# megvii-research/basedet

Measured on AMD Instinct MI355X. Metric: images/sec training RetinaNet-R50-FPN 1333x800, higher is better.
Workload: dtype bf16; 1 GPU; retinanet_r50_800x1344 train step (fwd+bwd+allreduce+SGD), DummyLoader boxes, random-init weights, inputs resident in HBM; per_gpu_batch=16, global_batch=16, parallelism=dp1

## Files before the change

### basedet_amd/_lib.py

```python
import ctypes as C
import os

import torch

_HERE = os.path.dirname(os.path.abspath(__file__))
LIB_PATH = os.environ.get("BASEDET_HIP_LIB") or os.path.join(_HERE, "lib", "libbasedet_hip.so")

BD_MAX_SEGS = 8
ABI_VERSION = 112
EPI_RELU, EPI_ADD_BEFORE, EPI_ADD_AFTER, EPI_MASK, EPI_SPARSE = 1, 2, 4, 8, 16


class BasedetHipError(RuntimeError):
    pass


class ConvDesc(C.Structure):
    _fields_ = [
        ("N", C.c_int32), ("Cin", C.c_int32), ("Cout", C.c_int32), ("R", C.c_int32), ("S", C.c_int32),
        ("stride", C.c_int32), ("pad", C.c_int32), ("nseg", C.c_int32),
        ("Hi", C.c_int32 * BD_MAX_SEGS), ("Wi", C.c_int32 * BD_MAX_SEGS),
        ("Ho", C.c_int32 * BD_MAX_SEGS), ("Wo", C.c_int32 * BD_MAX_SEGS),
        ("in_off", C.c_int32 * BD_MAX_SEGS), ("out_off", C.c_int32 * BD_MAX_SEGS),
        ("in_pix_per_img", C.c_int32), ("out_pix_per_img", C.c_int32),
        ("route", C.c_int32 * 4), ("sr_seed", C.c_uint32),
        ("gskip", C.c_int32), ("gskip_ws", C.c_void_p), ("gskip_ws_bytes", C.c_size_t),
        ("gskip_gmap", C.c_void_p), ("gskip_gmap_bytes", C.c_size_t), ("gskip_dxmap", C.c_void_p), ("gskip_dxmap_bytes", C.c_size_t),
        ("gskip_dx_clean", C.c_int32),
        ("fwd_map", C.c_void_p), ("fwd_map_bytes", C.c_size_t), ("fwd_clean", C.c_int32),
    ]


class PackDesc(C.Structure):
    _fields_ = [("w", C.c_void_p), ("row_scale", C.c_void_p), ("w_fwd", C.c_void_p), ("w_dgrad", C.c_void_p),
                ("Cout", C.c_int32), ("RS", C.c_int32), ("Cin", C.c_int32), ("block_start", C.c_int32)]


class ImageDesc(C.Structure):
    _fields_ = [("offset", C.c_int64), ("src_h", C.c_int32), ("src_w", C.c_int32), ("dst_h", C.c_int32), ("dst_w", C.c_int32),
                ("flip", C.c_int32), ("reserved_", C.c_int32 * 1)]


_P, _I, _L, _F, _Z = C.c_void_p, C.c_int, C.c_int64, C.c_float, C.c_size_t
_D = C.POINTER(ConvDesc)

SIGNATURES = {
    "bd_last_error_string": (C.c_char_p, []),
    "bd_version": (_I, []),
    "bd_conv_last_kernel": (C.c_char_p, []),
    "bd_probe_mfma_rate": (_I, [C.c_double, C.POINTER(C.c_double), C.POINTER(C.c_double), _P]),
    "bd_probe_kernel_clock": (_I, [C.c_char_p, _I, C.POINTER(C.c_double), C.POINTER(C.c_double)]),
    "bd_conv2d_fwd": (_I, [_D, _P, _P, _P, _P, _P, _I, _P]),
    "bd_conv2d_dgrad": (_I, [_D, _P, _P, _P, _P, _P, _I, _P]),
    "bd_conv2d_dgrad_gskip_bytes": (_Z, [_D]),
    "bd_conv2d_gskip_map_bytes": (_Z, [_D, _I]),
    "bd_gskip_map_scan": (_I, [_D, _I, _P, _P, _Z, _P]),
    "bd_fwd_live_map_bytes": (_Z, [_D]),
    "bd_fwd_live_maps": (_I, [_D, _P, _I, _I, C.POINTER(C.c_void_p), _Z, _I, _P]),
    "bd_conv2d_fwd_bits": (_I, [_D, _P, _P, _P, _P, _P, _P, _I, _P]),
    "bd_conv2d_fwd_ex": (_I, [_D, _P, _P, _P, _P, _P, _P, _P, _F, _I, _P]),
    "bd_conv2d_dgrad_ex": (_I, [_D, _P, _P, _P, _P, _P, _P, _P, _F, _I, _P]),
    "bd_conv2d_dgrad_bits": (_I, [_D, _P, _P, _P, _P, _P, _I, _P]),
    "bd_conv2d_wgrad_workspace_bytes": (_Z, [_D]),
    "bd_conv2d_wgrad": (_I, [_D, _P, _P, _P, _P, _I, _P, _Z, _P]),
    "bd_conv2d_wgrad_bias_workspace_bytes": (_Z, [_D]),
    "bd_conv2d_wgrad_bias": (_I, [_D, _P, _P, _P, _P, _P, _I, _P, _Z, _P]),
    "bd_fpn_deconv_pack": (_I, [_P, _I, _P, _P, _P]),
    "bd_fpn_deconv_fwd": (_I, [_P, _P, _P, _P, _I, _I, _I, _I, _I, _I, _P]),
    "bd_fpn_deconv_dgrad": (_I, [_P, _P, _P, _P, _I, _I, _I, _I, _I, _I, _P]),
    "bd_fpn_deconv_wgrad_workspace_bytes": (_Z, [_I, _I, _I, _I]),
    "bd_fpn_deconv_wgrad": (_I, [_P, _P, _P, _I, _P, _Z, _I, _I, _I, _I, _I, _I, _P]),
    "bd_wgrad_queue_create": (_I, [_P]),
    "bd_wgrad_queue_destroy": (_I, [_P]),
    "bd_wgrad_queue_pending": (_I, [_P]),
    "bd_conv2d_wgrad_queued": (_I, [_P, _D, _P, _P, _P, _P, _P, _I, _P, _Z, _P]),
    "bd_wgrad_queue_flush": (_I, [_P, _P]),
    "bd_stem_conv7x7_fwd": (_I, [_I, _I, _I, _P, _P, _P, _P, _P]),
    "bd_stem_conv7x7_raw_fwd": (_I, [_I, _I, _I, _P, _P, _P, _P]),
    "bd_stem_pool_fwd": (_I, [_I, _I, _I, _P, _P, _P, _P, _P]),
    "bd_stem_weight_pack": (_I, [_P, _P, _P, _P]),
    "bd_maxpool3x3s2_bwd": (_I, [_P, _P, _P, _I, _I, _I, _I, _P, _P]),
    "bd_stem_conv7x7_wgrad_workspace_bytes": (_Z, [_I, _I, _I]),
    "bd_stem_conv7x7_wgrad": (_I, [_I, _I, _I, _P, _P, _P, _P, _I, _P, _Z, _P]),
    "bd_weight_pack": (_I, [_P, _P, _P, _P, _I, _I, _I, _P]),
    "bd_weight_pack_blocks": (_I, [_I, _I, _I]),
    "bd_weight_pack_multi": (_I, [_P, _I, _I, _P]),
    "bd_colsum_workspace_bytes": (_Z, [_I]),
    "bd_colsum_bf16": (_I, [_P, _I, _L, _L, _L, _I, _P, _I, _P, _Z, _P]),
    "bd_pad_normalize": (_I, [_P, _I, _I, _I, _I, _I, _P, _P, _P, _P]),
    "bd_bottleneck_fwd_supported": (_I, [_I, _I, _I, _I, _I, _I, _I]),
    "bd_bottleneck_fwd": (_I, [_I, _I, _I, _I, _I, _I, _P, _P, _P, _P, _P, _P, _P, _P, _P, _P, _P]),
    "bd_h2d_create": (_I, [C.POINTER(C.c_void_p), _I, _I]),
    "bd_h2d_threads": (_I, [_P]),
    "bd_h2d_submit": (_I, [_P, _P, _I, _L, _P, _L, _P]),
    "bd_h2d_destroy": (_I, [_P]),
    "bd_pad_normalize_nchw": (_I, [_P, _I, _I, _I, _I, _I, _P, _P, _P, _P]),
    "bd_resize_pad_normalize": (_I, [_P, _L, C.POINTER(ImageDesc), _I, _I, _I, _P, _P, _P, _P]),
    "bd_maxpool3x3s2_fwd": (_I, [_P, _I, _I, _I, _I, _P, _P]),
    "bd_upsample2x_add_fwd": (_I, [_P, _L, _L, _P, _L, _L, _I, _I, _I, _I, _P]),
    "bd_upsample2x_add_bwd": (_I, [_P, _L, _L, _P, _L, _L, _I, _I, _I, _I, _I, _P]),
    "bd_relu_bf16": (_I, [_P, _P, _L, _P]),
    "bd_relu_bwd_bf16": (_I, [_P, _P, _P, _P, _L, _P]),
    "bd_add_bf16": (_I, [_P, _P, _P, _L, _P]),
    "bd_anchors_generate": (_I, [_I, _I, _I, _F, _P, _I, _P, _P]),
    "bd_points_generate": (_I, [_I, _I, _I, _F, _I, _P, _P]),
    "bd_box_pairwise": (_I, [_P, _I, _P, _I, _I, _P, _P]),
    "bd_box_encode": (_I, [_P, _P, _L, _P, _P, _P, _P]),
    "bd_box_decode": (_I, [_P, _P, _L, _P, _P, _P, _P]),
    "bd_retina_assign_encode": (_I, [_P, _I, _P, _P, _I, _I, _F, _F, _I, _P, _P, _P, _P, _P, _P, _P, _Z, _P]),
    "bd_fcos_assign": (_I, [_P, _I, _P, _P, _P, _I, _F, _P, _P, _I, _I, _P, _P, _P, _P, _P]),
    "bd_ota_assign_workspace_bytes": (_Z, [_I, _I]),
    "bd_ota_assign": (_I, [_P, _I, _P, _P, _I, _P, _I, _I, _P, _P, _P, _I, _I, _F, _F, _F, _F, _I, _P, _P, _P, _P, _P, _Z, _P]),
    "bd_ota_sinkhorn_workspace_bytes": (_Z, [_I, _I, _I]),
    "bd_ota_assign_sinkhorn": (_I, [_P, _I, _P, _P, _I, _P, _I, _I, _P, _P, _P, _I, _I, _F, _F, _F, _F, _I, _F, _I, _P, _P, _P, _P, _P, _Z, _P]),
    "bd_freeanchor_workspace_bytes": (_Z, [_I, _I, _I, _I]),
    "bd_freeanchor_loss_fwd_bwd": (_I, [_P, _I, _P, _I, _I, _P, _I, _I, _P, _P, _I, _I, _P, _P, _F, _I, _F, _F, _F, _F, _P, _P, _P, _P, _Z, _P]),
    "bd_atss_assign_workspace_bytes": (_Z, [_I, _I]),
    "bd_atss_assign": (_I, [_P, _I, _P, _P, _I, _I, _F, _P, _P, _I, _I, _P, _P, _P, _P, _P, _Z, _P]),
    "bd_nms_workspace_bytes": (_Z, [_I]),
    "bd_batched_nms": (_I, [_P, _P, _P, _I, _F, _I, _P, _P, _P, _Z, _P]),
    "bd_focal_loss_fwd_bwd": (_I, [_P, _P, _L, _I, _I, _F, _F, _P, _I, _F, _P, _P, _I, _P]),
    "bd_smooth_l1_fwd_bwd": (_I, [_P, _P, _P, _L, _I, _I, _F, _P, _I, _F, _P, _P, _P]),
    "bd_loss_grid_cap": (_I, []),
    "bd_iou_ltrb_fwd_bwd": (_I, [_P, _P, _P, _P, _L, _I, _P, _F, _P, _P, _P]),
    "bd_bce_logits_fwd_bwd": (_I, [_P, _I, _I, _P, _P, _L, _P, _P, _P, _P]),
    "bd_groupnorm_workspace_bytes": (_Z, [_I, _I, _I, _L]),
    "bd_groupnorm_fwd": (_I, [_P, _P, _P, _I, _I, _P, _P, _L, _I, _F, _I, _P, _P, _P, _Z, _P]),
    "bd_conv2d_fwd_gnstats_bytes": (_Z, [_D]),
    "bd_conv2d_fwd_gnstats": (_I, [_D, _P, _P, _P, _P, _P, _Z, _P]),
    "bd_groupnorm_fwd_parts": (_I, [_D, _P, _P, _P, _P, _F, _I, _P, _P, _P]),
    "bd_groupnorm_bwd": (_I, [_P, _P, _P, _P, _P, _I, _I, _P, _P, _L, _I, _I, _P, _P, _P, _I, _P, _Z, _P]),
    "bd_bn_workspace_bytes": (_Z, [_L, _I]),
    "bd_bn_stats_fwd": (_I, [_P, _I, _L, _L, _L, _I, _F, _F, _P, _P, _P, _P, _P, _P, _Z, _P]),
    "bd_bn_apply_act_fwd": (_I, [_P, _L, _L, _P, _P, _P, _P, _P, _L, _L, _P, _L, _L, _I, _L, _I, _I, _P]),
    "bd_bn_bwd_reduce": (_I, [_P, _L, _L, _P, _L, _L, _P, _P, _I, _L, _I, _P, _P, _P, _Z, _P]),
    "bd_bn_bwd_apply": (_I, [_P, _L, _L, _P, _L, _L, _P, _P, _P, _P, _P, _P, _P, _L, _L, _I, _L, _I, _P]),
    "bd_fcos_offsets_fwd": (_I, [_P, _I, _P, _I, _I, _P, _P, _P, _L, _P, _P]),
    "bd_fcos_offsets_workspace_bytes": (_Z, []),
    "bd_fcos_offsets_bwd": (_I, [_P, _I, _P, _I, _I, _P, _P, _P, _L, _P, _P, _P, _P, _P, _Z, _P]),
    "bd_rpn_assign_encode": (_I, [_P, _I, _P, _P, _I, _I, _F, _F, _I, _P, _P, _P, _P, _P, _P, _P, _Z, _P]),
    "bd_sample_labels": (_I, [_P, _P, _P, _I, _I, _I, _I, _P, _P]),
    "bd_segment_topk": (_I, [_P, _I, _I, _L, _I, _I, _I, _I, _P, _P, _I, _F, _I, _P, _P, _P, _P]),
    "bd_nms_batched_workspace_bytes": (_Z, [_I, _I]),
    "bd_nms_batched": (_I, [_P, _P, _P, _I, _I, _F, _I, _I, _P, _P, _P, _Z, _P]),
    "bd_rpn_proposals_workspace_bytes": (_Z, [_I, _I, _P, _I, _I, _I]),
    "bd_rpn_proposals": (_I, [_P, _I, _I, _I, _I, _I, _L, _I, _P, _P, _P, _P, _I, _P, _P, _I, _F, _I, _P, _P, _P, _Z, _I, _P]),
    "bd_rcnn_sample_targets": (_I, [_P, _P, _I, _P, _P, _I, _I, _P, _P, _I, _I, _I, _F, _F, _F, _P, _P, _P, _P, _P, _P, _P, _P]),
    "bd_roi_align_fwd": (_I, [_P, _L, _I, _I, _P, _P, _P, _P, _P, _P, _I, _I, _I, _I, _I, _P, _P]),
    "bd_conv1x1_thin_bwd_workspace_bytes": (_Z, []),
    "bd_conv1x1_thin_fwd": (_I, [_P, _P, _P, _L, _I, _I, _P, _P]),
    "bd_conv1x1_thin_bwd": (_I, [_P, _P, _P, _L, _I, _I, _P, _P, _P, _I, _P, _Z, _P]),
    "bd_roi_align_bwd": (_I, [_P, _L, _I, _I, _P, _P, _P, _P, _P, _P, _I, _I, _I, _I, _I, _P, _P]),
    "bd_roi_align_bwd_bf16_workspace_bytes": (_Z, [_I, _I, _P, _P, _I]),
    "bd_roi_align_bwd_bf16": (_I, [_P, _L, _I, _I, _I, _P, _P, _P, _P, _P, _P, _I, _I, _I, _I, _I, _P, _I, _P, _Z, _P]),
    "bd_roi_pool_fwd": (_I, [_P, _L, _I, _I, _P, _P, _P, _P, _P, _P, _I, _I, _I, _I, _P, _P]),
    "bd_roi_pool_bwd_bf16_workspace_bytes": (_Z, [_I, _I, _P, _P, _I]),
    "bd_roi_pool_bwd_bf16": (_I, [_P, _P, _L, _I, _I, _I, _P, _P, _P, _P, _P, _P, _I, _I, _I, _I, _P, _I, _P, _Z, _P]),
    "bd_subsample2x_fwd": (_I, [_P, _L, _L, _I, _I, _P, _L, _L, _I, _I, _P]),
    "bd_subsample2x_bwd_add": (_I, [_P, _L, _L, _P, _L, _L, _I, _I, _I, _I, _P]),
    "bd_f32_to_bf16": (_I, [_P, _P, _L, _P]),
    "bd_f32_to_bf16_add": (_I, [_P, _P, _L, _P]),
    "bd_rpn_loss_fwd_bwd": (_I, [_P, _I, _I, _I, _I, _P, _P, _L, _F, _P, _P, _P, _P]),
    "bd_rcnn_loss_fwd_bwd": (_I, [_P, _I, _I, _I, _P, _P, _I, _F, _P, _P, _P, _P]),
    "bd_det_scores": (_I, [_P, _I, _P, _I, _I, _L, _I, _P, _P]),
    "bd_det_select_workspace_bytes": (_Z, [_I, _I, _L, _I, _I]),
    "bd_det_select": (_I, [_P, _I, _P, _I, _I, _I, _L, _I, _I, _P, _P, _I, _F, _P, _P, _P, _P, _Z, _P]),
    "bd_rcnn_predict": (_I, [_P, _I, _I, _I, _P, _P, _I, _I, _P, _P, _P, _P, _P]),
    "bd_det_candidates": (_I, [_I, _P, _P, _P, _I, _I, _I, _P, _I, _P, _P, _L, _I, _I, _P, _P, _P, _L, _P, _P, _P, _P]),
    "bd_det_finalize": (_I, [_P, _P, _P, _P, _P, _I, _I, _I, _P, _I, _P, _P, _P, _P]),
    "bd_sgd_momentum_step": (_I, [_P, _P, _P, _L, _F, _F, _F, _F, _P]),
    "bd_ema_update": (_I, [_P, _P, _L, _F, _F, _P]),
    "bd_sgd_momentum_ema_step": (_I, [_P, _P, _P, _P, _L, _F, _F, _F, _F, _F, _F, _P]),
    "bd_swap_f32": (_I, [_P, _P, _L, _P]),
    "bd_adam_step": (_I, [_P, _P, _P, _P, _L] + [_F] * 10 + [_I, _P]),
# ... 93 lines not shown
```

### basedet_amd/csrc/bottleneck_fused.hip

```cpp
#include "common.h"

namespace {

constexpr int PH = 8, PW = 16;
constexpr int HH = PH + 2, HW = PW + 2;
constexpr int NHALO = HH * HW;
constexpr int NHP = 192;
constexpr int PITCH = 144;
constexpr int XB_BYTES = NHP * PITCH;
constexpr int W3_BYTES = 256 * PITCH;
constexpr int CMID = 64, COUT = 256;
constexpr unsigned X_NONE = 0x80000000u;

#ifdef BD_BN_STAMP
__device__ unsigned long long g_bn_stamp[16];
#define BN_STAMP(i) do { if (blockIdx.x == 0 && tid == 0 && tile_seq == 1) g_bn_stamp[i] = __builtin_amdgcn_s_memtime(); } while (0)
#else
#define BN_STAMP(i) do { } while (0)
#endif

struct BP {
    const bf16_raw *x, *w1, *w2, *w3, *wd;
    const float *b1, *b2, *b3, *bd;
    bf16_raw* y;
// ... 244 lines not shown
            for (int i = 0; i < NST; ++i) asm volatile("" : "+v"(st[a][i]));
#pragma unroll
        for (int hf = 0; hf < 2; ++hf)
#pragma unroll
        for (int half = 0; half < 2; ++half) {
            const int cbase = cb * 64 + 32 * half + 8 * q;
            const f32x4_t bv0 = *reinterpret_cast<const f32x4_t*>(B3L + cbase);
            const f32x4_t bv1 = *reinterpret_cast<const f32x4_t*>(B3L + cbase + 4);
            f32x4_t acc3[2][4], accd[2][4];
#pragma unroll
            for (int r = 0; r < 4; ++r) {
                acc3[0][r] = (f32x4_t){0.f, 0.f, 0.f, 0.f}; acc3[1][r] = (f32x4_t){0.f, 0.f, 0.f, 0.f};
                accd[0][r] = (f32x4_t){0.f, 0.f, 0.f, 0.f}; accd[1][r] = (f32x4_t){0.f, 0.f, 0.f, 0.f};
            }
#pragma unroll
            for (int ks = 0; ks < 2; ++ks) {
                bf16x8_t a[2], b[4];
#pragma unroll
                for (int t = 0; t < 2; ++t) a[t] = ld_frag_lds(W3L + (cb * 64 + (2 * half + t) * 16 + pxc) * PITCH + (ks ? xq1 : xq0));
#pragma unroll
                for (int r = 0; r < 4; ++r) b[r] = ld_frag_lds(M1 + ((hf * 4 + r) * 16 + pxc) * PITCH + (ks ? xq1 : xq0));
#pragma unroll
                for (int t = 0; t < 2; ++t)
#pragma unroll
                    for (int r = 0; r < 4; ++r) acc3[t][r] = __builtin_amdgcn_mfma_f32_16x16x32_bf16(a[t], b[r], acc3[t][r], 0, 0, 0);
                if constexpr (HAS_DS) {
#pragma unroll
                    for (int t = 0; t < 2; ++t) a[t] = ld_frag_lds(WDL + (cb * 64 + (2 * half + t) * 16 + pxc) * PITCH + (ks ? xq1 : xq0));
#pragma unroll
                    for (int r = 0; r < 4; ++r)
                        b[r] = ld_frag_lds(XB + xbuf * XB_BYTES + ((hf * 4 + r + 1) * HW + 1 + pxc) * PITCH + (ks ? xq1 : xq0));
#pragma unroll
                    for (int t = 0; t < 2; ++t)
#pragma unroll
                        for (int r = 0; r < 4; ++r) accd[t][r] = __builtin_amdgcn_mfma_f32_16x16x32_bf16(a[t], b[r], accd[t][r], 0, 0, 0);
                }
            }
            [[maybe_unused]] f32x4_t dv0, dv1;
            if constexpr (HAS_DS) {
                dv0 = *reinterpret_cast<const f32x4_t*>(B3L + 256 + cbase);
                dv1 = *reinterpret_cast<const f32x4_t*>(B3L + 256 + cbase + 4);
            }
#pragma unroll
            for (int r = 0; r < 4; ++r) {
                u32x4_t o;
#pragma unroll
                for (int k = 0; k < 4; ++k) {
                    const f32x4_t bk = (k >> 1) ? bv1 : bv0;
                    f32x2_bn_t v = {acc3[k >> 1][r][2 * (k & 1)], acc3[k >> 1][r][2 * (k & 1) + 1]};
                    v += (f32x2_bn_t){bk[2 * (k & 1)], bk[2 * (k & 1) + 1]};
                    if constexpr (!HAS_DS) {
                        const unsigned w = res_all[hf][half][r][k];
                        v += (f32x2_bn_t){bf_lo(w), bf_hi(w)};
                    } else {
                        const f32x4_t dk = (k >> 1) ? dv1 : dv0;
                        f32x2_bn_t d = {accd[k >> 1][r][2 * (k & 1)], accd[k >> 1][r][2 * (k & 1) + 1]};
                        d += (f32x2_bn_t){dk[2 * (k & 1)], dk[2 * (k & 1) + 1]};
                        const unsigned w = __builtin_bit_cast(unsigned, __builtin_convertvector(d, bf16x2_bn_t));
                        v += (f32x2_bn_t){bf_lo(w), bf_hi(w)};
                    }
                    o[k] = relu_pack2(v[0], v[1]);
                }
                __builtin_amdgcn_raw_buffer_store_b128(o, y_rsrc, yoff[hf * 4 + r], 64 * half, 0);
            }
        }

        BN_STAMP(5);
        ++tile_seq;
        if (!have_next) break;
        tile = next_tile;
#pragma unroll
        for (int i = 0; i < NST; ++i) voff[i] = nvoff[i];
        n_img = nn; ty0 = ny0; tx0 = nx0;
        next_tile = tile + stride;
        have_next = next_tile < t_end;
        if (have_next) decode(next_tile, nvoff, nn, ny0, nx0);
        if constexpr (NCH == 1) {
            if (have_next) { if ((g & 1) == 0) stage_load(st[0], nvoff, 0); else stage_load(st[1], nvoff, 0); }
            g ^= 1;
        }
    }
}

}

#ifdef BD_BN_STAMP
extern "C" int bd_debug_bn_stamp(unsigned long long* out16) {
    return hipMemcpyFromSymbol(out16, HIP_SYMBOL(g_bn_stamp), sizeof(g_bn_stamp)) == hipSuccess ? 0 : 1;
}
#endif

extern "C" int bd_bottleneck_fwd_supported(int N, int H, int W, int Cin, int Cmid, int Cout, int has_ds) {
    if (N < 1 || H < 1 || W < 1) return 0;
    if (Cmid != CMID || Cout != COUT) return 0;
    if (!((Cin == 64 && has_ds) || (Cin == 256 && !has_ds))) return 0;
    const long long bytes_in = (long long)N * H * W * Cin * 2, bytes_out = (long long)N * H * W * Cout * 2;
    return bytes_in < 0x7fffffffll && bytes_out < 0x7fffffffll;
}

extern "C" int bd_bottleneck_fwd(int N, int H, int W, int Cin, int Cmid, int Cout, const void* x, const void* w1, const float* b1,
                                 const void* w2, const float* b2, const void* w3, const float* b3, const void* wd, const float* bd,
                                 void* y, bd_stream_t stream) {
    BD_REQUIRE(x && w1 && b1 && w2 && b2 && w3 && b3 && y, "bottleneck_fwd: null pointer");
    BD_REQUIRE(bd_bottleneck_fwd_supported(N, H, W, Cin, Cmid, Cout, wd != nullptr), "bottleneck_fwd: unsupported shape N=%d %dx%d %d->%d->%d ds=%d",
               N, H, W, Cin, Cmid, Cout, wd != nullptr);
    BD_REQUIRE(wd == nullptr || bd != nullptr, "bottleneck_fwd: downsample weights without their shift");
    BP p{};
    p.x = (const bf16_raw*)x; p.w1 = (const bf16_raw*)w1; p.w2 = (const bf16_raw*)w2; p.w3 = (const bf16_raw*)w3; p.wd = (const bf16_raw*)wd;
    p.b1 = b1; p.b2 = b2; p.b3 = b3; p.bd = bd; p.y = (bf16_raw*)y;
    p.N = N; p.H = H; p.W = W;
    p.tiles_x = cdiv(W, PW);
    p.tiles_y = cdiv(H, PH);
    p.tiles_per_img = p.tiles_x * p.tiles_y;
    p.total_tiles = p.tiles_per_img * N;
    p.per_xcd = cdiv(p.total_tiles, 8);
    p.x_bytes = (unsigned)((long long)N * H * W * Cin * 2);
    p.y_bytes = (unsigned)((long long)N * H * W * Cout * 2);
    const int cus = bd_num_cus();
    int grid = (cus / 8) * 8;
    if (grid < 8) grid = 8;
    const int need = p.per_xcd * 8;
    if (grid > need) grid = need;
    const size_t lds = 2 * XB_BYTES + XB_BYTES + W3_BYTES + (wd ? W3_BYTES : 0) + BIAS_BYTES + PAD_BYTES;
    BD_ONCE_PER_DEVICE(
        (void)hipFuncSetAttribute(reinterpret_cast<const void*>(&bottleneck_fused_kernel<64, true>), hipFuncAttributeMaxDynamicSharedMemorySize,
                                  3 * XB_BYTES + 2 * W3_BYTES + BIAS_BYTES + PAD_BYTES);
        (void)hipFuncSetAttribute(reinterpret_cast<const void*>(&bottleneck_fused_kernel<256, false>), hipFuncAttributeMaxDynamicSharedMemorySize,
                                  3 * XB_BYTES + W3_BYTES + BIAS_BYTES + PAD_BYTES));
    if (wd) hipLaunchKernelGGL((bottleneck_fused_kernel<64, true>), dim3(grid), dim3(256), lds, (hipStream_t)stream, p);
    else hipLaunchKernelGGL((bottleneck_fused_kernel<256, false>), dim3(grid), dim3(256), lds, (hipStream_t)stream, p);
    BD_CHECK_LAUNCH("bd_bottleneck_fwd");
    return BD_OK;
}
```

### basedet_amd/ops.py

```python
import ctypes as C
from dataclasses import dataclass, field
from typing import List, Optional

import torch

from . import _lib
from ._lib import ConvDesc, EPI_ADD_AFTER, EPI_ADD_BEFORE, EPI_MASK, EPI_RELU, EPI_SPARSE, check, f32arr, i32arr, ptr, stream_ptr


@dataclass
class Geom:
    N: int
    H: List[int]
    W: List[int]
    off: List[int] = field(default_factory=list)
    pix_per_img: int = 0

    def __post_init__(self):
        if not self.off:
            o = 0
            self.off = []
            for h, w in zip(self.H, self.W):
                self.off.append(o)
                o += h * w
# ... 850 lines not shown
    def __init__(self):
        self._h = C.c_void_p()
        check(L().bd_wgrad_queue_create(C.byref(self._h)), "bd_wgrad_queue_create")

    def wgrad(self, d, x, g, dw, dbias, ws, row_scale=None, accumulate=False):
        check(L().bd_conv2d_wgrad_queued(self._h, C.byref(_stamp(d)), ptr(x), ptr(g), ptr(row_scale), ptr(dw), ptr(dbias), int(accumulate), ptr(ws),
                                         ws.numel() * ws.element_size(), stream_ptr()), "bd_conv2d_wgrad_queued")

    def pending(self):
        return int(L().bd_wgrad_queue_pending(self._h))

    def flush(self):
        check(L().bd_wgrad_queue_flush(self._h, stream_ptr()), "bd_wgrad_queue_flush")

    def close(self):
        if self._h:
            L().bd_wgrad_queue_destroy(self._h)
            self._h = C.c_void_p()

    def __del__(self):
        try:
            self.close()
        except Exception:
            pass


def clip_grad_value(g, lower, upper, pre_scale=1.0):
    check(L().bd_clip_grad_value(ptr(g), g.numel(), float(pre_scale), float(lower), float(upper), stream_ptr()), "bd_clip_grad_value")


def clip_grad_norm_workspace_bytes():
    return int(L().bd_clip_grad_norm_workspace_bytes())


def clip_grad_norm(g, max_norm, ord=2.0, pre_scale=1.0, norm_out=None, ws=None):
    if ws is None:
        ws = torch.empty((clip_grad_norm_workspace_bytes(),), dtype=torch.uint8, device=g.device)
    check(L().bd_clip_grad_norm(ptr(g), g.numel(), float(pre_scale), float(max_norm), float(ord), ptr(norm_out), ptr(ws), ws.numel(),
                                stream_ptr()), "bd_clip_grad_norm")
    return norm_out


class HostStager:

    _DT = {"float64": 0, "float32": 1, "uint8": 2}

    def __init__(self, device, threads=0):
        self._h = C.c_void_p()
        self.device = torch.device(device)
        index = self.device.index if self.device.index is not None else torch.cuda.current_device()
        self.device = torch.device("cuda", index)
        check(L().bd_h2d_create(C.byref(self._h), int(index), int(threads)), "bd_h2d_create")
        self.threads = int(L().bd_h2d_threads(self._h))

    def supports(self, arr):
        return hasattr(arr, "dtype") and str(arr.dtype) in self._DT and getattr(arr, "flags", None) is not None and arr.flags["C_CONTIGUOUS"]

    def submit(self, arr, out=None, chunk_elems=0):
        if out is None:
            out = torch.empty(arr.shape, dtype=torch.float32, device=self.device)
        assert out.is_contiguous() and out.numel() == arr.size and out.dtype == torch.float32
        check(L().bd_h2d_submit(self._h, C.c_void_p(arr.ctypes.data), self._DT[str(arr.dtype)], arr.size, ptr(out), int(chunk_elems),
                                stream_ptr()), "bd_h2d_submit")
        return out

    def close(self):
        if self._h:
            L().bd_h2d_destroy(self._h)
            self._h = C.c_void_p()

    def __del__(self):
        try:
            self.close()
        except Exception:
            pass


def bottleneck_fwd_supported(N, H, W, cin, cmid, cout, has_ds):
    return bool(L().bd_bottleneck_fwd_supported(int(N), int(H), int(W), int(cin), int(cmid), int(cout), int(bool(has_ds))))


def bottleneck_fwd(N, H, W, cin, cmid, cout, x, w1, b1, w2, b2, w3, b3, wd, bd, y):
    check(L().bd_bottleneck_fwd(int(N), int(H), int(W), int(cin), int(cmid), int(cout), ptr(x), ptr(w1), ptr(b1), ptr(w2), ptr(b2),
                                ptr(w3), ptr(b3), ptr(wd), ptr(bd), ptr(y), stream_ptr()), "bd_bottleneck_fwd")
    return y
```

### include/basedet_hip.h

```cpp
#ifndef BASEDET_HIP_H
#define BASEDET_HIP_H

#include <stddef.h>
#include <stdint.h>

#ifdef __cplusplus
extern "C" {
#endif

#define BD_OK 0
#define BD_EINVAL (-1)
#define BD_ELAUNCH (-2)
#define BD_EWORKSPACE (-3)

#define BD_MAX_SEGS 8

#define BD_EPI_RELU 1
#define BD_EPI_ADD_BEFORE 2
#define BD_EPI_ADD_AFTER 4
#define BD_EPI_MASK 8
#define BD_EPI_SPARSE 16

typedef void* bd_stream_t;

// ... 22 lines not shown
    int32_t fwd_clean;
} bd_conv_desc;

const char* bd_last_error_string(void);
int bd_version(void);
const char* bd_conv_last_kernel(void);
int bd_probe_mfma_rate(double seconds, double* tflops_out, double* clock_mhz_out, bd_stream_t stream);

int bd_probe_kernel_clock(const char* kernel, int reset, double* clock_mhz_out, double* busy_ms_out);


int bd_conv2d_fwd(const bd_conv_desc* d, const void* x, const void* w_packed, const float* bias,
                  const void* add, void* y, int flags, bd_stream_t stream);

int bd_conv2d_dgrad(const bd_conv_desc* d, const void* g, const void* w_packed_t, const void* add,
                    const void* mask, void* dx, int flags, bd_stream_t stream);
size_t bd_conv2d_dgrad_gskip_bytes(const bd_conv_desc* d);
size_t bd_conv2d_gskip_map_bytes(const bd_conv_desc* d, int of_dx);
int bd_gskip_map_scan(const bd_conv_desc* d, int of_dx, const void* t, void* map, size_t map_bytes, bd_stream_t stream);
size_t bd_fwd_live_map_bytes(const bd_conv_desc* d);
int bd_fwd_live_maps(const bd_conv_desc* d, const int32_t* labels, int A, int depths, void* const* maps, size_t map_bytes, int reset,
                     bd_stream_t stream);

int bd_conv2d_fwd_bits(const bd_conv_desc* d, const void* x, const void* w_packed, const float* bias, const void* add, void* y,
                       uint32_t* ybits, int flags, bd_stream_t stream);
int bd_conv2d_dgrad_bits(const bd_conv_desc* d, const void* g, const void* w_packed_t, const void* add, const uint32_t* maskbits,
                         void* dx, int flags, bd_stream_t stream);
int bd_conv2d_fwd_ex(const bd_conv_desc* d, const void* x, const void* w_packed, const float* bias, const void* add, void* y,
                     uint32_t* ybits, void* y8, float q_scale, int flags, bd_stream_t stream);
int bd_conv2d_dgrad_ex(const bd_conv_desc* d, const void* g, const void* w_packed_t, const void* add, const void* mask,
                       const uint32_t* maskbits, void* dx, void* dx8, float q_scale, int flags, bd_stream_t stream);

size_t bd_conv2d_wgrad_workspace_bytes(const bd_conv_desc* d);
int bd_conv2d_wgrad(const bd_conv_desc* d, const void* x, const void* g, const float* row_scale, float* dw,
                    int accumulate, void* ws, size_t ws_bytes, bd_stream_t stream);

size_t bd_conv2d_wgrad_bias_workspace_bytes(const bd_conv_desc* d);
int bd_conv2d_wgrad_bias(const bd_conv_desc* d, const void* x, const void* g, const float* row_scale, float* dw, float* dbias,
                         int accumulate, void* ws, size_t ws_bytes, bd_stream_t stream);

typedef struct bd_wgrad_queue* bd_wgrad_queue_t;
int bd_wgrad_queue_create(bd_wgrad_queue_t* out);
int bd_wgrad_queue_destroy(bd_wgrad_queue_t q);
int bd_wgrad_queue_pending(bd_wgrad_queue_t q);
int bd_conv2d_wgrad_queued(bd_wgrad_queue_t q, const bd_conv_desc* d, const void* x, const void* g, const float* row_scale, float* dw,
                           float* dbias, int accumulate, void* ws, size_t ws_bytes, bd_stream_t stream);
int bd_wgrad_queue_flush(bd_wgrad_queue_t q, bd_stream_t stream);



int bd_stem_conv7x7_fwd(int N, int H, int W, const void* x_halo, const void* w_stem, const float* bias,
                        void* y, bd_stream_t stream);
int bd_stem_conv7x7_raw_fwd(int N, int H, int W, const void* x_halo, const void* w_stem, void* y, bd_stream_t stream);
int bd_stem_pool_fwd(int N, int H, int W, const void* x_halo, const void* w_stem, const float* bias, void* y_pool,
                     bd_stream_t stream);
int bd_stem_weight_pack(const float* w , const float* row_scale, void* w_stem,
                        bd_stream_t stream);

int bd_maxpool3x3s2_bwd(const void* g_pool, const void* stem_out, const void* pool_out, int N, int Hs, int Ws, int C, void* g_stem,
                        bd_stream_t stream);
size_t bd_stem_conv7x7_wgrad_workspace_bytes(int N, int H, int W);
int bd_stem_conv7x7_wgrad(int N, int H, int W, const void* x_halo, const void* g_stem, const float* row_scale, float* dw, int accumulate,
                          void* ws, size_t ws_bytes, bd_stream_t stream);

int bd_weight_pack(const float* w, const float* row_scale, void* w_fwd, void* w_dgrad, int Cout, int RS,
                   int Cin, bd_stream_t stream);

typedef struct bd_pack_desc {
    const float* w;
    const float* row_scale;
    void* w_fwd;
    void* w_dgrad;
    int32_t Cout, RS, Cin, block_start;
} bd_pack_desc;
int bd_weight_pack_blocks(int Cout, int RS, int Cin);
int bd_weight_pack_multi(const bd_pack_desc* descs_dev, int n, int total_blocks, bd_stream_t stream);

size_t bd_colsum_workspace_bytes(int C);
int bd_colsum_bf16(const void* g, int N, int64_t pix_per_img, int64_t off, int64_t cnt, int C, float* out,
                   int accumulate, void* ws, size_t ws_bytes, bd_stream_t stream);

int bd_bottleneck_fwd_supported(int N, int H, int W, int Cin, int Cmid, int Cout, int has_downsample);
int bd_bottleneck_fwd(int N, int H, int W, int Cin, int Cmid, int Cout, const void* x, const void* w1, const float* b1, const void* w2,
                      const float* b2, const void* w3, const float* b3, const void* wd, const float* bd, void* y, bd_stream_t stream);


int bd_pad_normalize(const float* in, int N, int H, int W, int Hp, int Wp, const float* mean3,
                     const float* std3, void* out, bd_stream_t stream);
typedef struct bd_h2d* bd_h2d_t;
#define BD_HOST_F64 0
#define BD_HOST_F32 1
#define BD_HOST_U8 2
int bd_h2d_create(bd_h2d_t* out, int device, int threads);
int bd_h2d_threads(bd_h2d_t h);
int bd_h2d_submit(bd_h2d_t h, const void* src_host, int src_dtype, int64_t n, float* dst_dev, int64_t chunk_elems, bd_stream_t stream);
int bd_h2d_destroy(bd_h2d_t h);

int bd_pad_normalize_nchw(const float* in, int N, int H, int W, int Hp, int Wp, const float* mean3,
                          const float* std3, float* out, bd_stream_t stream);

typedef struct bd_image_desc {
    int64_t offset;
    int32_t src_h, src_w, dst_h, dst_w, flip;
    int32_t reserved_[1];
} bd_image_desc;
int bd_resize_pad_normalize(const uint8_t* packed_dev, int64_t packed_bytes, const bd_image_desc* descs_host, int N, int Hp, int Wp,
                            const float* mean3, const float* std3, void* x_halo, bd_stream_t stream);

int bd_maxpool3x3s2_fwd(const void* x, int N, int H, int W, int C, void* y, bd_stream_t stream);

int bd_upsample2x_add_fwd(const void* top, int64_t top_pix_per_img, int64_t top_off, void* lateral,
                          int64_t lat_pix_per_img, int64_t lat_off, int N, int H, int W, int C,
                          bd_stream_t stream);
int bd_upsample2x_add_bwd(const void* dlat, int64_t lat_pix_per_img, int64_t lat_off, void* dtop,
                          int64_t top_pix_per_img, int64_t top_off, int N, int H, int W, int C,
                          int accumulate, bd_stream_t stream);

int bd_fpn_deconv_pack(const float* w, int C, void* w_fwd, void* w_dgrad, bd_stream_t stream);
int bd_fpn_deconv_fwd(const void* x, const void* w_fwd, const void* add, void* y, int N, int Hc, int Wc, int Hf, int Wf, int C,
                      bd_stream_t stream);
int bd_fpn_deconv_dgrad(const void* dy, const void* w_dgrad, const void* add, void* dx, int N, int Hc, int Wc, int Hf, int Wf, int C,
                        bd_stream_t stream);
size_t bd_fpn_deconv_wgrad_workspace_bytes(int N, int Hc, int Wc, int C);
int bd_fpn_deconv_wgrad(const void* x, const void* dy, float* dw, int accumulate, void* ws, size_t ws_bytes, int N, int Hc, int Wc,
                        int Hf, int Wf, int C, bd_stream_t stream);

int bd_relu_bf16(const void* x, void* y, int64_t n, bd_stream_t stream);
int bd_relu_bwd_bf16(const void* g, const void* mask, const void* add, void* y, int64_t n, bd_stream_t stream);
int bd_add_bf16(const void* a, const void* b, void* y, int64_t n, bd_stream_t stream);


int bd_anchors_generate(int H, int W, int stride, float offset, const float* base, int A, float* out,
                        bd_stream_t stream);
int bd_points_generate(int H, int W, int stride, float offset, int A, float* out, bd_stream_t stream);

int bd_box_pairwise(const float* b1, int m, const float* b2, int n, int mode, float* out, bd_stream_t stream);

int bd_box_encode(const float* anchors, const float* gt, int64_t n, const float* mean4_host,
                  const float* std4_host, float* out, bd_stream_t stream);
int bd_box_decode(const float* anchors, const float* deltas, int64_t n, const float* mean4_host,
                  const float* std4_host, float* out, bd_stream_t stream);

int bd_retina_assign_encode(const float* anchors, int A, const float* gt_boxes, const int32_t* num_gt, int N,
                            int Gmax, float thr_lo, float thr_hi, int allow_low_quality,
                            const float* mean4_host, const float* std4_host, int32_t* labels,
                            int32_t* match_idx, float* offsets, int32_t* num_fg, void* ws, size_t ws_bytes,
                            bd_stream_t stream);

int bd_fcos_assign(const float* points, int P, const int32_t* lvl_start_host, const float* soi_host,
                   const int32_t* strides_host, int L, float radius, const float* gt_boxes,
                   const int32_t* num_gt, int N, int Gmax, int32_t* labels, float* offsets, float* ctrness,
                   float* stats, bd_stream_t stream);

size_t bd_atss_assign_workspace_bytes(int N, int P);
int bd_atss_assign(const float* points, int P, const int32_t* lvl_start_host, const int32_t* strides_host, int L, int topk,
                   float anchor_scale, const float* gt_boxes, const int32_t* num_gt, int N, int Gmax, int32_t* labels,
                   float* offsets, float* ctrness, float* stats, void* ws, size_t ws_bytes, bd_stream_t stream);

size_t bd_ota_assign_workspace_bytes(int N, int P);
int bd_ota_assign(const float* points, int P, const int32_t* lvl_start_host, const int32_t* strides_host, int L, const void* logits,
                  int K, int ld, const void* pred_ltrb, const float* gt_boxes, const int32_t* num_gt, int N, int Gmax, float alpha,
                  float gamma, float reg_weight, float center_radius, int candidate_k, int32_t* labels, float* targets,
                  float* gt_ious, float* stats, void* ws, size_t ws_bytes, bd_stream_t stream);

size_t bd_ota_sinkhorn_workspace_bytes(int N, int P, int Gmax);
int bd_ota_assign_sinkhorn(const float* points, int P, const int32_t* lvl_start_host, const int32_t* strides_host, int L,
                           const void* logits, int K, int ld, const void* pred_ltrb, const float* gt_boxes, const int32_t* num_gt,
// ... 251 lines not shown
```

Measured before the change: 727.4 images/sec.

## Add DMA-staged fused bottleneck kernel variant for layer1 non-downsample blocks

Adds a new fused layer1 bottleneck kernel for the 256-channel, no-downsample case. It stages halo input chunks straight into LDS with buffer DMA, double-buffers them, and prefetches the next tile's input during the 3x3 stage, with extra loads into a pad region to warm L2. It runs by default unless a route bit disables it, and the ABI gains a route argument. The aim is to hide input-load latency behind MFMA work and cut LDS use, at the cost of more complex synchronisation and a separate code path.

```diff
diff --git a/basedet_amd/_lib.py b/basedet_amd/_lib.py
--- a/basedet_amd/_lib.py
+++ b/basedet_amd/_lib.py
@@ -89,7 +89,7 @@
     "bd_colsum_bf16": (_I, [_P, _I, _L, _L, _L, _I, _P, _I, _P, _Z, _P]),
     "bd_pad_normalize": (_I, [_P, _I, _I, _I, _I, _I, _P, _P, _P, _P]),
     "bd_bottleneck_fwd_supported": (_I, [_I, _I, _I, _I, _I, _I, _I]),
-    "bd_bottleneck_fwd": (_I, [_I, _I, _I, _I, _I, _I, _P, _P, _P, _P, _P, _P, _P, _P, _P, _P, _P]),
+    "bd_bottleneck_fwd": (_I, [_I, _I, _I, _I, _I, _I, _P, _P, _P, _P, _P, _P, _P, _P, _P, _P, _I, _P]),
     "bd_h2d_create": (_I, [C.POINTER(C.c_void_p), _I, _I]),
     "bd_h2d_threads": (_I, [_P]),
     "bd_h2d_submit": (_I, [_P, _P, _I, _L, _P, _L, _P]),
diff --git a/basedet_amd/csrc/bottleneck_fused.hip b/basedet_amd/csrc/bottleneck_fused.hip
--- a/basedet_amd/csrc/bottleneck_fused.hip
+++ b/basedet_amd/csrc/bottleneck_fused.hip
@@ -350,6 +350,237 @@
     }
 }
 
+struct BnDma {};
+constexpr int XD_BYTES = NHALO * PITCH;
+constexpr int XD_UNITS = NHALO * 9;
+constexpr int NTD = 512;
+constexpr int NDM = 4;
+constexpr int DMA_LDS_BYTES = 2 * XD_BYTES + XB_BYTES + W3_BYTES + BIAS_BYTES;
+static_assert(NHALO * PITCH + 1024 <= XB_BYTES, "the L2 warm-up pad lies in mid-1 rows 180..191");
+
+template <typename STAGE, int CIN>
+__global__ __launch_bounds__(NTD, 1) void bottleneck_fused_kernel(const BP p) {
+    static_assert(CIN == 256, "blocks 1 and 2 of layer1");
+    constexpr int NCH = CIN / 64;
+    extern __shared__ __attribute__((aligned(16))) unsigned char smem[];
+    unsigned char* const XB = smem;
+    unsigned char* const M1 = smem + 2 * XD_BYTES;
+    unsigned char* const W3L = M1 + XB_BYTES;
+    float* const B3L = reinterpret_cast<float*>(W3L + W3_BYTES);
+    unsigned char* const PAD = M1 + NHALO * PITCH;
+
+    const int tid = threadIdx.x, lane = tid & 63;
+    const int wave = __builtin_amdgcn_readfirstlane(tid >> 6);
+    const int px = lane & 15, q = lane >> 4;
+    const int pxc = colperm(px);
+    const int xq0 = xpos(q), xq1 = xpos(q + 4);
+    const int cb = wave & 3, ph = wave >> 2;
+    const int wq = xpos(cb * 2 + (q >> 1)) + (q & 1) * 8;
+
+    bf16x8_t w1r[2 * NCH], w2r[18];
+    {
+        const bf16_raw* r1 = p.w1 + (long long)(cb * 16 + px) * CIN + q * 8;
+#pragma unroll
+        for (int s = 0; s < 2 * NCH; ++s) w1r[s] = *reinterpret_cast<const bf16x8_t*>(r1 + s * 32);
+        const bf16_raw* r2 = p.w2 + (long long)(cb * 16 + px) * 576 + q * 8;
+#pragma unroll
+        for (int s = 0; s < 18; ++s) w2r[s] = *reinterpret_cast<const bf16x8_t*>(r2 + s * 32);
+    }
+    for (int u = tid; u < 256 * 8; u += NTD) {
+        const int row = u >> 3, part = u & 7;
+        const int t = (row >> 4) & 3, rho = colperm_inv(row & 15);
+        const int ch = (row & ~63) + 32 * (t >> 1) + 8 * (rho >> 2) + 4 * (t & 1) + (rho & 3);
+        *reinterpret_cast<u32x4_t*>(W3L + row * PITCH + xpos(part)) = *reinterpret_cast<const u32x4_t*>(p.w3 + (long long)ch * CMID + part * 8);
+    }
+    if (tid < 256) B3L[tid] = p.b3[tid];
+    else if (tid < 256 + CMID) B3L[tid] = p.b1[tid - 256];
+    else if (tid < 256 + 2 * CMID) B3L[tid] = p.b2[tid - 256 - CMID];
+
+    const __amdgpu_buffer_rsrc_t x_rsrc = __builtin_amdgcn_make_buffer_rsrc(const_cast<bf16_raw*>(p.x), 0, p.x_bytes, 0x00020000);
+    const __amdgpu_buffer_rsrc_t y_rsrc = __builtin_amdgcn_make_buffer_rsrc(p.y, 0, p.y_bytes, 0x00020000);
+
+    const int xcd = blockIdx.x & 7, slot = blockIdx.x >> 3, stride = gridDim.x >> 3;
+    const int t_end = min((xcd + 1) * p.per_xcd, p.total_tiles);
+    int tile = xcd * p.per_xcd + slot;
+
+    auto decode = [&](int t, unsigned (&vo)[NDM], int& n, int& y0, int& x0) {
+        n = t / p.tiles_per_img;
+        const int r = t - n * p.tiles_per_img;
+        const int ty = r / p.tiles_x;
+        y0 = ty * PH; x0 = (r - ty * p.tiles_x) * PW;
+        int tt = tid;
+        asm volatile("" : "+v"(tt));
+#pragma unroll
+        for (int i = 0; i < NDM; ++i) {
+            const int u = tt + NTD * i, h = u / 9, part = u - 9 * h;
+            const int hy = h / HW, hx = h - hy * HW;
+            const int chunk = (part & 4) | ((part & 1) << 1) | ((part >> 1) & 1);
+            const int gy = y0 - 1 + hy, gx = x0 - 1 + hx;
+            const bool ok = part < 8 && h < NHALO && gy >= 0 && gy < p.H && gx >= 0 && gx < p.W;
+            vo[i] = ok ? (unsigned)((((long long)n * p.H + gy) * p.W + gx) * CIN + chunk * 8) * 2u : X_NONE;
+        }
+    };
+    auto dma_chunk = [&](unsigned char* dst, const unsigned (&vo)[NDM], int c) {
+        int so = c * 128;
+        asm volatile("" : "+s"(so));
+#pragma unroll
+        for (int i = 0; i < NDM - 1; ++i) dma16_bn(x_rsrc, dst + i * (NTD * 16), vo[i], so);
+        if (tid + NTD * (NDM - 1) < XD_UNITS) dma16_bn(x_rsrc, dst + (NDM - 1) * (NTD * 16), vo[NDM - 1], so);
+    };
+    unsigned char* const xdst0 = XB + wave * 1024;
+    unsigned char* const xdst1 = XB + XD_BYTES + wave * 1024;
+
+    if (tile >= t_end) return;
+    unsigned voff[NDM], nvoff[NDM];
+    int n_img = 0, ty0 = 0, tx0 = 0, nn = 0, ny0 = 0, nx0 = 0;
+    decode(tile, voff, n_img, ty0, tx0);
+    dma_chunk(xdst0, voff, 0);
+    dma_chunk(xdst1, voff, 1);
+    int next_tile = tile + stride;
+    bool have_next = next_tile < t_end;
+    if (have_next) decode(next_tile, nvoff, nn, ny0, nx0);
+    asm volatile("s_waitcnt vmcnt(0)" ::: "memory");
+    [[maybe_unused]] int tile_seq = 0;
+
+    for (;;) {
+        BN_STAMP(0);
+        f32x4_t acc1[6];
+#pragma unroll
+        for (int j = 0; j < 6; ++j) acc1[j] = (f32x4_t){0.f, 0.f, 0.f, 0.f};
+#pragma unroll
+        for (int c = 0; c < NCH; ++c) {
+            if (c >= 2) asm volatile("s_waitcnt vmcnt(0)" ::: "memory");
+            __syncthreads();
+            if (c == 1) dma_chunk(xdst0, voff, 2);
+            if (c == 2) dma_chunk(xdst1, voff, 3);
+            const unsigned char* xb = XB + (c & 1) * XD_BYTES + (ph * 96 + pxc) * PITCH;
+#pragma unroll
+            for (int ks = 0; ks < 2; ++ks)
+#pragma unroll
+                for (int j = 0; j < 6; ++j)
+                    acc1[j] = __builtin_amdgcn_mfma_f32_16x16x32_bf16(w1r[c * 2 + ks], ld_frag_lds(xb + j * 16 * PITCH + (ks ? xq1 : xq0)), acc1[j], 0, 0, 0);
+        }
+        BN_STAMP(1);
+        const f32x4_t b1v = *reinterpret_cast<const f32x4_t*>(B3L + 256 + cb * 16 + 4 * q);
+#pragma unroll
+        for (int j = 0; j < 6; ++j) {
+            const int h = (ph * 6 + j) * 16 + pxc, hy = h / HW, hx = h - hy * HW;
+            const int gy = ty0 - 1 + hy, gx = tx0 - 1 + hx;
+            const bool in = gy >= 0 && gy < p.H && gx >= 0 && gx < p.W;
+            u32x2_t o;
+            const f32x4_t v = acc1[j] + b1v;
+            o[0] = in ? relu_pack2(v[0], v[1]) : 0u;
+            o[1] = in ? relu_pack2(v[2], v[3]) : 0u;
+            *reinterpret_cast<u32x2_t*>(M1 + h * PITCH + wq) = o;
+        }
+        __syncthreads();
+
+        BN_STAMP(2);
+        if (have_next) {
+            dma_chunk(xdst0, nvoff, 0);
+            dma_chunk(xdst1, nvoff, 1);
+#pragma unroll
+            for (int c = 2; c < NCH; ++c) {
+                int so = c * 128;
+                asm volatile("" : "+s"(so));
+#pragma unroll
+                for (int i = 0; i < NDM - 1; ++i) dma16_bn(x_rsrc, PAD, nvoff[i], so);
+                if (tid + NTD * (NDM - 1) < XD_UNITS) dma16_bn(x_rsrc, PAD, nvoff[NDM - 1], so);
+            }
+        }
+
+        f32x4_t acc2[4];
+#pragma unroll
+        for (int r = 0; r < 4; ++r) acc2[r] = (f32x4_t){0.f, 0.f, 0.f, 0.f};
+        {
+            const unsigned char* mb = M1 + (ph * 4 * HW + pxc) * PITCH;
+#pragma unroll
+            for (int t = 0; t < 9; ++t)
+#pragma unroll
+                for (int kh = 0; kh < 2; ++kh)
+#pragma unroll
+                    for (int r = 0; r < 4; ++r)
+                        acc2[r] = __builtin_amdgcn_mfma_f32_16x16x32_bf16(
+                            w2r[t * 2 + kh], ld_frag_lds(mb + ((r + t / 3) * HW + t % 3) * PITCH + (kh ? xq1 : xq0)), acc2[r], 0, 0, 0);
+        }
+        BN_STAMP(3);
+        asm volatile("s_waitcnt vmcnt(0)" ::: "memory");
+        __syncthreads();
+        const f32x4_t b2v = *reinterpret_cast<const f32x4_t*>(B3L + 256 + CMID + cb * 16 + 4 * q);
+#pragma unroll
+        for (int r = 0; r < 4; ++r) {
+            u32x2_t o;
+            const f32x4_t v = acc2[r] + b2v;
+            o[0] = relu_pack2(v[0], v[1]);
+            o[1] = relu_pack2(v[2], v[3]);
+            *reinterpret_cast<u32x2_t*>(M1 + ((ph * 4 + r) * 16 + pxc) * PITCH + wq) = o;
+        }
+        u32x4_t res[2][4];
+        auto res_load = [&](u32x4_t (&rr)[4], int half) {
+#pragma unroll
+            for (int r = 0; r < 4; ++r) {
+                const int gy = ty0 + ph * 4 + r, gx = tx0 + pxc;
+                const bool ok = gy < p.H && gx < p.W;
+                const unsigned vo = ok ? (unsigned)((((long long)n_img * p.H + gy) * p.W + gx) * CIN + cb * 64 + 32 * half + 8 * q) * 2u : X_NONE;
+                rr[r] = __builtin_amdgcn_raw_buffer_load_b128(x_rsrc, vo, 0, 0);
+            }
+        };
+        res_load(res[0], 0);
+        __syncthreads();
+
+        BN_STAMP(4);
+#pragma unroll
+        for (int half = 0; half < 2; ++half) {
+            const int cbase = cb * 64 + 32 * half + 8 * q;
+            const f32x4_t bv0 = *reinterpret_cast<const f32x4_t*>(B3L + cbase);
+            const f32x4_t bv1 = *reinterpret_cast<const f32x4_t*>(B3L + cbase + 4);
+            f32x4_t acc3[2][4];
+#pragma unroll
+            for (int r = 0; r < 4; ++r) { acc3[0][r] = (f32x4_t){0.f, 0.f, 0.f, 0.f}; acc3[1][r] = (f32x4_t){0.f, 0.f, 0.f, 0.f}; }
+#pragma unroll
+            for (int ks = 0; ks < 2; ++ks) {
+                bf16x8_t a[2], b[4];
+#pragma unroll
+                for (int t = 0; t < 2; ++t) a[t] = ld_frag_lds(W3L + (cb * 64 + (2 * half + t) * 16 + pxc) * PITCH + (ks ? xq1 : xq0));
+#pragma unroll
+                for (int r = 0; r < 4; ++r) b[r] = ld_frag_lds(M1 + ((ph * 4 + r) * 16 + pxc) * PITCH + (ks ? xq1 : xq0));
+#pragma unroll
+                for (int t = 0; t < 2; ++t)
+#pragma unroll
+                    for (int r = 0; r < 4; ++r) acc3[t][r] = __builtin_amdgcn_mfma_f32_16x16x32_bf16(a[t], b[r], acc3[t][r], 0, 0, 0);
+            }
+            if (half == 0) res_load(res[1], 1);
+#pragma unroll
+            for (int r = 0; r < 4; ++r) {
+                u32x4_t o;
+#pragma unroll
+                for (int k = 0; k < 4; ++k) {
+                    const f32x4_t bk = (k >> 1) ? bv1 : bv0;
+                    f32x2_bn_t v = {acc3[k >> 1][r][2 * (k & 1)], acc3[k >> 1][r][2 * (k & 1) + 1]};
+                    v += (f32x2_bn_t){bk[2 * (k & 1)], bk[2 * (k & 1) + 1]};
+                    const unsigned w = res[half][r][k];
+                    v += (f32x2_bn_t){bf_lo(w), bf_hi(w)};
+                    o[k] = relu_pack2(v[0], v[1]);
+                }
+                const int gy = ty0 + ph * 4 + r, gx = tx0 + pxc;
+                const unsigned yo = (gy < p.H && gx < p.W) ? (unsigned)((((long long)n_img * p.H + gy) * p.W + gx) * COUT + cb * 64 + 8 * q) * 2u : X_NONE;
+                __builtin_amdgcn_raw_buffer_store_b128(o, y_rsrc, yo, 64 * half, 0);
+            }
+        }
+
+        BN_STAMP(5);
+        ++tile_seq;
+        if (!have_next) break;
+        tile = next_tile;
+#pragma unroll
+        for (int i = 0; i < NDM; ++i) voff[i] = nvoff[i];
+        n_img = nn; ty0 = ny0; tx0 = nx0;
+        next_tile = tile + stride;
+        have_next = next_tile < t_end;
+        if (have_next) decode(next_tile, nvoff, nn, ny0, nx0);
+    }
+}
+
 }
 
 #ifdef BD_BN_STAMP
@@ -368,7 +599,7 @@
 
 extern "C" int bd_bottleneck_fwd(int N, int H, int W, int Cin, int Cmid, int Cout, const void* x, const void* w1, const float* b1,
                                  const void* w2, const float* b2, const void* w3, const float* b3, const void* wd, const float* bd,
-                                 void* y, bd_stream_t stream) {
+                                 void* y, int route, bd_stream_t stream) {
     BD_REQUIRE(x && w1 && b1 && w2 && b2 && w3 && b3 && y, "bottleneck_fwd: null pointer");
     BD_REQUIRE(bd_bottleneck_fwd_supported(N, H, W, Cin, Cmid, Cout, wd != nullptr), "bottleneck_fwd: unsupported shape N=%d %dx%d %d->%d->%d ds=%d",
                N, H, W, Cin, Cmid, Cout, wd != nullptr);
@@ -384,11 +615,20 @@
     p.per_xcd = cdiv(p.total_tiles, 8);
     p.x_bytes = (unsigned)((long long)N * H * W * Cin * 2);
     p.y_bytes = (unsigned)((long long)N * H * W * Cout * 2);
+    BD_REQUIRE(route >= 0, "bottleneck_fwd: negative route word (0 = the library's choice, otherwise the bd_conv_desc.route[1] mask + 1)");
+    const bool dma = !wd && !(route && (((route - 1) >> 15) & 1));
     const int cus = bd_num_cus();
     int grid = (cus / 8) * 8;
     if (grid < 8) grid = 8;
     const int need = p.per_xcd * 8;
     if (grid > need) grid = need;
+    if (dma) {
+        BD_ONCE_PER_DEVICE((void)hipFuncSetAttribute(reinterpret_cast<const void*>(&bottleneck_fused_kernel<BnDma, 256>),
+                                                     hipFuncAttributeMaxDynamicSharedMemorySize, DMA_LDS_BYTES));
+        hipLaunchKernelGGL((bottleneck_fused_kernel<BnDma, 256>), dim3(grid), dim3(NTD), DMA_LDS_BYTES, (hipStream_t)stream, p);
+        BD_CHECK_LAUNCH("bd_bottleneck_fwd");
+        return BD_OK;
+    }
     const size_t lds = 2 * XB_BYTES + XB_BYTES + W3_BYTES + (wd ? W3_BYTES : 0) + BIAS_BYTES + PAD_BYTES;
     BD_ONCE_PER_DEVICE(
         (void)hipFuncSetAttribute(reinterpret_cast<const void*>(&bottleneck_fused_kernel<64, true>), hipFuncAttributeMaxDynamicSharedMemorySize,
diff --git a/basedet_amd/ops.py b/basedet_amd/ops.py
--- a/basedet_amd/ops.py
+++ b/basedet_amd/ops.py
@@ -956,5 +956,5 @@
 
 def bottleneck_fwd(N, H, W, cin, cmid, cout, x, w1, b1, w2, b2, w3, b3, wd, bd, y):
     check(L().bd_bottleneck_fwd(int(N), int(H), int(W), int(cin), int(cmid), int(cout), ptr(x), ptr(w1), ptr(b1), ptr(w2), ptr(b2),
-                                ptr(w3), ptr(b3), ptr(wd), ptr(bd), ptr(y), stream_ptr()), "bd_bottleneck_fwd")
-    return y
+                                ptr(w3), ptr(b3), ptr(wd), ptr(bd), ptr(y), _ROUTE[1], stream_ptr()), "bd_bottleneck_fwd")
+    return y
diff --git a/include/basedet_hip.h b/include/basedet_hip.h
--- a/include/basedet_hip.h
+++ b/include/basedet_hip.h
@@ -128,7 +128,8 @@
 
 int bd_bottleneck_fwd_supported(int N, int H, int W, int Cin, int Cmid, int Cout, int has_downsample);
 int bd_bottleneck_fwd(int N, int H, int W, int Cin, int Cmid, int Cout, const void* x, const void* w1, const float* b1, const void* w2,
-                      const float* b2, const void* w3, const float* b3, const void* wd, const float* bd, void* y, bd_stream_t stream);
+                      const float* b2, const void* w3, const float* b3, const void* wd, const float* bd, void* y, int route,
+                      bd_stream_t stream);
 
 
 int bd_pad_normalize(const float* in, int N, int H, int W, int Hp, int Wp, const float* mean3,
```

Result: no change. 730.3 images/sec, median of 6 (+0.4%).
